# SnakeOnex/vit-is-all-you-need

Measured on AMD Instinct MI355X. Metric: images/sec ViT-B/16 224px bf16 fwd+bwd, higher is better.
Workload: dtype bf16; 1 GPU; ViT-B/16 224x224 bf16 forward+loss+backward, batch 256 per GPU (BASELINE configs[1]; configs[2] at 8 GPUs), random-init weights, 197 tokens, 79.44 M params; global_batch=256, parallelism=dp1

## Files before the change

vit-is-all-you-need_amd/csrc/attention.hip:

```cpp
#include "common.h"
#include "vitamd_internal.h"
#include <type_traits>

namespace {

constexpr int DH = 64;
constexpr int MAX_N = 512;
constexpr int MAX_N_LONG = 16384;
constexpr float NEG_BIG = -1.0e30f;

typedef LDS_AS bf16x4* lds_bf16x4_ptr;

__device__ __forceinline__ int swz(int row) { return (((row >> 1) & 1) << 2) | ((row >> 3) & 3); }

__device__ __forceinline__ void stage_tile(const __bf16* __restrict__ g, int ld, int N, int npad, char* lds, int wave, int lane, int nwaves = 4) {
  const int pieces = npad / 8;
  for (int pc = wave; pc < pieces; pc += nwaves) {
    const int row = pc * 8 + (lane >> 3);
    const int logical = (lane & 7) ^ swz(row);
    const int grow = min(row, N - 1);
    glds16(g + (size_t)grow * ld + logical * 8, lds + pc * 1024);
  }
}

__device__ __forceinline__ bf16x8 row_frag(const char* tile, int T, int kk, int lane) {
  const int rr = lane & 31;
  const int chunk = (2 * kk + (lane >> 5)) ^ swz(rr);
  return *(const bf16x8*)(tile + T * 4096 + rr * 128 + (chunk << 4));
}

__device__ __forceinline__ bf16x8 tr_frag(const char* tile, int T, int s, int dt, int lane) {
  const int h = lane >> 5, colhalf = (lane >> 4) & 1, qq = (lane >> 2) & 3, pp = lane & 3;
  const int chunk = 4 * dt + 2 * colhalf + (pp >> 1);
  bf16x4 part[2];
#pragma unroll
  for (int u = 0; u < 2; ++u) {
    const int rloc = 16 * s + 8 * u + 4 * h + qq;
    const int f = (((qq >> 1) & 1) << 2) | (2 * s + u);
    part[u] = __builtin_amdgcn_ds_read_tr16_b64_v4bf16((lds_bf16x4_ptr)(tile + T * 4096 + rloc * 128 + ((chunk ^ f) << 4) + (pp & 1) * 8));
  }
  return __builtin_shufflevector(part[0], part[1], 0, 1, 2, 3, 4, 5, 6, 7);
}

__device__ __forceinline__ bf16x8 acc_to_frag(const f32x16& x, int s) {
  bf16x8 f;
#pragma unroll
  for (int j = 0; j < 8; ++j) f[j] = (__bf16)x[8 * s + j];
  return f;
}

__device__ __forceinline__ void zero(f32x16& x) {
#pragma unroll
  for (int r = 0; r < 16; ++r) x[r] = 0.f;
}
__device__ __forceinline__ void zero(f32x16 (&x)[2]) {
#pragma unroll
  for (int dt = 0; dt < 2; ++dt) zero(x[dt]);
}

__device__ __forceinline__ void load_lane_frags(const __bf16* __restrict__ g, int ld, int N, int r0, int lane, bf16x8 (&f)[4]) {
  const int row = min(r0 + (lane & 31), N - 1);
  const __bf16* p = g + (size_t)row * ld + 8 * (lane >> 5);
#pragma unroll
  for (int kk = 0; kk < 4; ++kk) f[kk] = *(const bf16x8*)(p + 16 * kk);
}

__device__ __forceinline__ int acc_row(int reg, int lane) { return (reg & 3) + 8 * (reg >> 2) + 4 * (lane >> 5); }
__device__ __forceinline__ float fast_exp2(float x) { return __builtin_amdgcn_exp2f(x); }
__device__ __forceinline__ float max16(const f32x16& v) {
  float a = fmaxf(fmaxf(v[0], v[1]), fmaxf(v[2], v[3])), b = fmaxf(fmaxf(v[4], v[5]), fmaxf(v[6], v[7]));
  float c = fmaxf(fmaxf(v[8], v[9]), fmaxf(v[10], v[11])), d = fmaxf(fmaxf(v[12], v[13]), fmaxf(v[14], v[15]));
  return fmaxf(fmaxf(a, b), fmaxf(c, d));
}

__device__ __forceinline__ void store_rows_T(__bf16* __restrict__ g, int ld, int N, int r0, int lane, const f32x16 (&acc)[2], float scale) {
  const int row = r0 + (lane & 31);
  if (row >= N) return;
  __bf16* p = g + (size_t)row * ld + 4 * (lane >> 5);
#pragma unroll
  for (int dt = 0; dt < 2; ++dt)
#pragma unroll
    for (int u = 0; u < 4; ++u) {
      u32x2 o = {pack_bf16x2(acc[dt][4 * u] * scale, acc[dt][4 * u + 1] * scale),
                 pack_bf16x2(acc[dt][4 * u + 2] * scale, acc[dt][4 * u + 3] * scale)};
      *(u32x2*)(p + 32 * dt + 8 * u) = o;
    }
}

template <int ROWS = 32, bool RES = false>
__device__ __forceinline__ void store_rows_T_img(__bf16* __restrict__ g, int ld, int N, int r0, int lane, const f32x16 (&acc)[2], float scale, char* img,
                                                 float* colacc = nullptr, const float* __restrict__ xi = nullptr, float* __restrict__ xo = nullptr,
                                                 int ldx = 0) {
  const int rr = lane & 31, h = lane >> 5;
  constexpr int ITS = ROWS / 8;
  int pass = 0;
#pragma unroll
  do {
    f32x4 r[ITS][2];
    if constexpr (RES) {
#pragma unroll
      for (int it = 0; it < ITS; ++it) {
        const int row = (lane >> 3) + 8 * it, pc = lane & 7;
        const float* px = xi + (size_t)min(r0 + ROWS * pass + row, N - 1) * ldx + 8 * (pc ^ (row & 7));
        r[it][0] = *(const f32x4*)px;
        r[it][1] = *(const f32x4*)(px + 4);
      }
    }
    if (ROWS == 32 || (rr >> 4) == pass) {
#pragma unroll
      for (int dt = 0; dt < 2; ++dt)
#pragma unroll
        for (int u = 0; u < 4; ++u) {
          u32x2 o = {pack_bf16x2(acc[dt][4 * u] * scale, acc[dt][4 * u + 1] * scale),
                     pack_bf16x2(acc[dt][4 * u + 2] * scale, acc[dt][4 * u + 3] * scale)};
          *(u32x2*)(img + (rr & (ROWS - 1)) * 128 + (((4 * dt + u) ^ (rr & 7)) << 4) + h * 8) = o;
        }
    }
#pragma unroll
    for (int it = 0; it < ITS; ++it) {
      const int row = (lane >> 3) + 8 * it, pc = lane & 7;
      const u32x4 v = *(const u32x4*)(img + row * 128 + pc * 16);
      const int grow = r0 + ROWS * pass + row;
      if (grow < N) {
        const int col = 8 * (pc ^ (row & 7));
        *(u32x4*)(g + (size_t)grow * ld + col) = v;
        if constexpr (RES) {
          f32x4 o0 = {r[it][0][0] + bf16lo(v[0]), r[it][0][1] + bf16hi(v[0]), r[it][0][2] + bf16lo(v[1]), r[it][0][3] + bf16hi(v[1])};
          f32x4 o1 = {r[it][1][0] + bf16lo(v[2]), r[it][1][1] + bf16hi(v[2]), r[it][1][2] + bf16lo(v[3]), r[it][1][3] + bf16hi(v[3])};
          float* po = xo + (size_t)grow * ldx + col;
          *(f32x4*)po = o0;
          *(f32x4*)(po + 4) = o1;
        }
      }
    }
  } while (ROWS == 16 && ++pass < 2);
  if constexpr (ROWS == 32) {
    if (colacc) {
      const int chunk = lane >> 3, within = (lane & 7) * 2;
      const int nrows = min(32, N - r0);
      float sacc = 0.f;
      for (int row = 0; row < nrows; ++row)
        sacc += bf2f(*(const __bf16*)(img + row * 128 + ((chunk ^ (row & 7)) << 4) + within));
      *colacc += sacc;
    }
  }
}

struct AttnArgs {
  const __bf16* qkv;
  __bf16* o;
  float* lse2;
  const __bf16* d_o;
  __bf16* dqkv;
  float* delta;
  float* dbias;
  int B, N, H;
  int causal;
  float scale_log2e;
  float scale;
  unsigned drop_thresh;
  float drop_scale;
  unsigned seed_lo, seed_hi;
  const float* resid_in;
  float* resid_out;
  int nq;
};

struct HeadAddr {
  int b, hh, N, D3, D;
  const __bf16* qbase;
};
template <typename Idx>
__device__ __forceinline__ HeadAddr head_addr(const __bf16* qkv, int N, int H, Idx head) {
  const int b = head / H, hh = head % H, D3 = 3 * H * DH, D = H * DH;
  return {b, hh, N, D3, D, qkv + (size_t)b * N * D3 + hh * DH};
}
__device__ __forceinline__ size_t stat_index(int b, int H, int hh, int N, int row) { return ((size_t)b * H + hh) * N + row; }

__device__ __forceinline__ float attn_keep(const AttnArgs& a, int bh, int query, int key) {
  const unsigned long long idx = ((unsigned long long)bh * a.N + query) * a.N + key;
  return dropout_keep(idx, a.seed_lo, a.seed_hi, a.drop_thresh, a.drop_scale);
}

template <bool DROP>
__global__ __launch_bounds__(256) void attn_fwd_kernel(const AttnArgs a) {
  extern __shared__ __attribute__((aligned(16))) char smem[];
  const int lane = threadIdx.x & 63, wave = __builtin_amdgcn_readfirstlane(threadIdx.x >> 6);
  const auto [b, hh, N, D3, D, qbase] = head_addr(a.qkv, a.N, a.H, blockIdx.x);
  const int nt = (N + 31) / 32, npad = nt * 32;
  char* ktile = smem;
  char* vtile = smem + npad * 128;
  stage_tile(qbase + D, D3, N, npad, ktile, wave, lane);
  stage_tile(qbase + 2 * D, D3, N, npad, vtile, wave, lane);
  asm volatile("s_waitcnt vmcnt(0)" ::: "memory");
  __syncthreads();

  const float c = a.scale_log2e;
  for (int qb = wave; qb < nt; qb += 4) {
    const int q0 = qb * 32;
    const int qrow = q0 + (lane & 31);
    bf16x8 qf[4];
    load_lane_frags(qbase, D3, N, q0, lane, qf);
    f32x16 oacc[2];
    zero(oacc);
    float m = NEG_BIG, l = 0.f;
    const int t_end = a.causal ? min(nt, qb + 1) : nt;
    for (int T = 0; T < t_end; ++T) {
      f32x16 s;
      zero(s);
#pragma unroll
      for (int kk = 0; kk < 4; ++kk) s = __builtin_amdgcn_mfma_f32_32x32x16_bf16(row_frag(ktile, T, kk, lane), qf[kk], s, 0, 0, 0);
      if (32 * T + 32 > N || (a.causal && T == qb)) {
#pragma unroll
        for (int r = 0; r < 16; ++r) {
          const int key = 32 * T + acc_row(r, lane);
          if (!(key < N && (!a.causal || key <= qrow))) s[r] = NEG_BIG;
        }
      }
      float tmax = max16(s);
      tmax = fmaxf(tmax, __shfl_xor(tmax, 32, 64)) * c;
      const float mnew = fmaxf(m, tmax);
      const float alpha = fast_exp2(m - mnew);
      m = mnew;
      float psum = 0.f;
#pragma unroll
      for (int r = 0; r < 16; ++r) {
        s[r] = fast_exp2(__builtin_fmaf(s[r], c, -mnew));
        psum += s[r];
        if constexpr (DROP) s[r] *= attn_keep(a, blockIdx.x, min(qrow, N - 1), min(32 * T + acc_row(r, lane), N - 1));
      }
      l = l * alpha + psum;
#pragma unroll
      for (int dt = 0; dt < 2; ++dt)
#pragma unroll
        for (int r = 0; r < 16; ++r) oacc[dt][r] *= alpha;
#pragma unroll
      for (int sidx = 0; sidx < 2; ++sidx) {
        const bf16x8 pf = acc_to_frag(s, sidx);
#pragma unroll
        for (int dt = 0; dt < 2; ++dt)
          oacc[dt] = __builtin_amdgcn_mfma_f32_32x32x16_bf16(tr_frag(vtile, T, sidx, dt, lane), pf, oacc[dt], 0, 0, 0);
      }
    }
    l += __shfl_xor(l, 32, 64);
    const float inv = 1.0f / l;
    store_rows_T(a.o + (size_t)b * N * D + hh * DH, D, N, q0, lane, oacc, inv);
    if (lane < 32 && qrow < N) a.lse2[stat_index(b, a.H, hh, N, qrow)] = m + log2f(l);
  }
}

template <int NKT, bool DROP, bool CAUSAL, bool RES = false>
__global__ __launch_bounds__(256, 2) void attn_fwd_small_kernel(const AttnArgs a) {
  extern __shared__ __attribute__((aligned(16))) char smem[];
  const int lane = threadIdx.x & 63, wave = __builtin_amdgcn_readfirstlane(threadIdx.x >> 6);
  const int head = blockIdx.x;
  const auto [b, hh, N, D3, D, qbase] = head_addr(a.qkv, a.N, a.H, head);
  constexpr int nt = NKT, npad = NKT * 32;
  char* ktile = smem;
  char* vtile = smem + npad * 128;
  char* oimg = smem + 2 * npad * 128 + wave * 4096;
  stage_tile(qbase + D, D3, N, npad, ktile, wave, lane);
  stage_tile(qbase + 2 * D, D3, N, npad, vtile, wave, lane);
  const int wrot = (wave + head) & 3;
  bf16x8 qf[4], qf2[4];
  load_lane_frags(qbase, D3, N, wrot * 32, lane, qf);
  if (wrot + 4 < nt) load_lane_frags(qbase, D3, N, wrot * 32 + 128, lane, qf2);
  else {
#pragma unroll
    for (int kk = 0; kk < 4; ++kk) qf2[kk] = qf[kk];
  }
  asm volatile("s_waitcnt vmcnt(0)" ::: "memory");
#pragma unroll
  for (int kk = 0; kk < 4; ++kk) asm volatile("" : "+v"(qf[kk]), "+v"(qf2[kk]));
  __syncthreads();

  const float c = a.scale_log2e;
  for (int qb = wrot; qb < nt; qb += 4) {
    const int q0 = qb * 32;
    const int qrow = q0 + (lane & 31);
    if (qb != wrot) {
#pragma unroll
      for (int kk = 0; kk < 4; ++kk) qf[kk] = qf2[kk];
    }
    const int t_end = CAUSAL ? qb + 1 : nt;
    f32x16 s[NKT];
    float mx = NEG_BIG;
#pragma unroll
    for (int T = 0; T < NKT; ++T) {
      if (T < t_end) {
#pragma unroll
        for (int r = 0; r < 16; ++r) s[T][r] = 0.f;
#pragma unroll
        for (int kk = 0; kk < 4; ++kk) s[T] = __builtin_amdgcn_mfma_f32_32x32x16_bf16(row_frag(ktile, T, kk, lane), qf[kk], s[T], 0, 0, 0);
        if (32 * T + 32 > N || (CAUSAL && T == qb)) {
#pragma unroll
          for (int r = 0; r < 16; ++r) {
            const int key = 32 * T + acc_row(r, lane);
            if (!(key < N && (!CAUSAL || key <= qrow))) s[T][r] = NEG_BIG;
          }
        }
        mx = fmaxf(mx, max16(s[T]));
      }
    }
    mx = fmaxf(mx, __shfl_xor(mx, 32, 64));
    const float mc = mx * c;
    float l = 0.f;
    f32x16 oacc[2];
#pragma unroll
    for (int dt = 0; dt < 2; ++dt)
#pragma unroll
      for (int r = 0; r < 16; ++r) oacc[dt][r] = 0.f;
#pragma unroll
    for (int T = 0; T < NKT; ++T) {
      if (T < t_end) {
#pragma unroll
        for (int r = 0; r < 16; ++r) {
          float pexp = fast_exp2(__builtin_fmaf(s[T][r], c, -mc));
          l += pexp;
          if constexpr (DROP) pexp *= attn_keep(a, head, min(qrow, N - 1), min(32 * T + acc_row(r, lane), N - 1));
          s[T][r] = pexp;
        }
#pragma unroll
        for (int sidx = 0; sidx < 2; ++sidx) {
          const bf16x8 pf = acc_to_frag(s[T], sidx);
#pragma unroll
          for (int dt = 0; dt < 2; ++dt)
            oacc[dt] = __builtin_amdgcn_mfma_f32_32x32x16_bf16(tr_frag(vtile, T, sidx, dt, lane), pf, oacc[dt], 0, 0, 0);
        }
      }
    }
    l += __shfl_xor(l, 32, 64);
    const float inv = 1.0f / l;
    if constexpr (RES)
      store_rows_T_img<32, true>(a.o + (size_t)b * N * D + hh * DH, D, N, q0, lane, oacc, inv, oimg, nullptr, a.resid_in + (size_t)b * N * D + hh * DH,
                                 a.resid_out + (size_t)b * N * D + hh * DH, D);
    else
      store_rows_T_img(a.o + (size_t)b * N * D + hh * DH, D, N, q0, lane, oacc, inv, oimg);
    if (lane < 32 && qrow < N) a.lse2[stat_index(b, a.H, hh, N, qrow)] = mc + log2f(l);
  }
}

template <int NKT, bool RES, bool KEEP = false>
__global__ __launch_bounds__(512, 4) void attn_fwd_small8_kernel(const AttnArgs a) {
  extern __shared__ __attribute__((aligned(16))) char smem[];
  const int lane = threadIdx.x & 63, wave = __builtin_amdgcn_readfirstlane(threadIdx.x >> 6);
  const int head = blockIdx.x;
  const auto [b, hh, N, D3, D, qbase] = head_addr(a.qkv, a.N, a.H, head);
  constexpr int nt = NKT, npad = NKT * 32;
  char* ktile = smem;
  char* vtile = smem + npad * 128;
  char* oimg = smem + 2 * npad * 128 + wave * 2048;
  stage_tile(qbase + D, D3, N, npad, ktile, wave, lane, 8);
  stage_tile(qbase + 2 * D, D3, N, npad, vtile, wave, lane, 8);
  const int qb = (wave + head) & 7;
  bool active = qb < nt;
  if constexpr (KEEP) active = qb * 32 < a.nq;
  bf16x8 qf[4];
  load_lane_frags(qbase, D3, N, (active ? qb : 0) * 32, lane, qf);
  asm volatile("s_waitcnt vmcnt(0)" ::: "memory");
#pragma unroll
  for (int kk = 0; kk < 4; ++kk) asm volatile("" : "+v"(qf[kk]));
  __syncthreads();
  if (!active) return;
  const float c = a.scale_log2e;
  const int q0 = qb * 32;
  const int qrow = q0 + (lane & 31);
  float m = NEG_BIG, l = 0.f;
  f32x16 oacc[2];
  zero(oacc);
#pragma unroll 1
  for (int T = 0; T < NKT; ++T) {
    f32x16 st;
    zero(st);
#pragma unroll
    for (int kk = 0; kk < 4; ++kk) st = __builtin_amdgcn_mfma_f32_32x32x16_bf16(row_frag(ktile, T, kk, lane), qf[kk], st, 0, 0, 0);
    if (32 * T + 32 > N) {
#pragma unroll
      for (int r = 0; r < 16; ++r)
        if (!(32 * T + acc_row(r, lane) < N)) st[r] = NEG_BIG;
    }
    float mt = max16(st);
    mt = fmaxf(mt, __shfl_xor(mt, 32, 64));
    const float mn = fmaxf(m, mt);
    const float alpha = fast_exp2((m - mn) * c);
    m = mn;
    const float mc = mn * c;
    float lt = 0.f;
#pragma unroll
    for (int r = 0; r < 16; ++r) {
      const float pexp = fast_exp2(__builtin_fmaf(st[r], c, -mc));
      lt += pexp;
      st[r] = pexp;
    }
    l = l * alpha + lt;
    if (T > 0) {
#pragma unroll
      for (int dt = 0; dt < 2; ++dt)
#pragma unroll
        for (int r = 0; r < 16; ++r) oacc[dt][r] *= alpha;
    }
#pragma unroll
    for (int sidx = 0; sidx < 2; ++sidx) {
      const bf16x8 pf = acc_to_frag(st, sidx);
#pragma unroll
      for (int dt = 0; dt < 2; ++dt)
        oacc[dt] = __builtin_amdgcn_mfma_f32_32x32x16_bf16(tr_frag(vtile, T, sidx, dt, lane), pf, oacc[dt], 0, 0, 0);
    }
  }
  l += __shfl_xor(l, 32, 64);
  const float mc = m * c;
  const float inv = 1.0f / l;
  if constexpr (KEEP) {
    store_rows_T_img<16>(a.o + (size_t)b * a.nq * D + hh * DH, D, a.nq, q0, lane, oacc, inv, oimg);
    if (lane < 32 && qrow < a.nq) a.lse2[stat_index(b, a.H, hh, N, qrow)] = mc + log2f(l);
    return;
  }
  if constexpr (RES)
    store_rows_T_img<16, true>(a.o + (size_t)b * N * D + hh * DH, D, N, q0, lane, oacc, inv, oimg, nullptr, a.resid_in + (size_t)b * N * D + hh * DH,
                               a.resid_out + (size_t)b * N * D + hh * DH, D);
  else
    store_rows_T_img<16>(a.o + (size_t)b * N * D + hh * DH, D, N, q0, lane, oacc, inv, oimg);
  if (lane < 32 && qrow < N) a.lse2[stat_index(b, a.H, hh, N, qrow)] = mc + log2f(l);
}

template <bool DROP, bool CAUSAL>
__global__ __launch_bounds__(256, 2) void attn_bwd_dq_kernel(const AttnArgs a) {
  extern __shared__ __attribute__((aligned(16))) char smem[];
  const int lane = threadIdx.x & 63, wave = __builtin_amdgcn_readfirstlane(threadIdx.x >> 6);
  const auto [b, hh, N, D3, D, qbase] = head_addr(a.qkv, a.N, a.H, blockIdx.x);
  const int nt = (N + 31) / 32, npad = nt * 32;
  char* ktile = smem;
  char* vtile = smem + npad * 128;
  char* oimg = smem + 2 * npad * 128 + wave * 4096;
  stage_tile(qbase + D, D3, N, npad, ktile, wave, lane);
  stage_tile(qbase + 2 * D, D3, N, npad, vtile, wave, lane);
  asm volatile("s_waitcnt vmcnt(0)" ::: "memory");
  __syncthreads();

  const float c = a.scale_log2e;
  const __bf16* obase = a.o + (size_t)b * N * D + hh * DH;
  const __bf16* dobase = a.d_o + (size_t)b * N * D + hh * DH;
  float csum_q = 0.f;
  for (int qb = (wave + blockIdx.x) & 3; qb < nt; qb += 4) {
    const int q0 = qb * 32;
    const int qrow = q0 + (lane & 31);
    bf16x8 qf[4], dof[4], of[4];
    load_lane_frags(qbase, D3, N, q0, lane, qf);
    load_lane_frags(dobase, D, N, q0, lane, dof);
    load_lane_frags(obase, D, N, q0, lane, of);
    float delta = 0.f;
#pragma unroll
    for (int kk = 0; kk < 4; ++kk)
#pragma unroll
      for (int j = 0; j < 8; ++j) delta += (float)dof[kk][j] * (float)of[kk][j];
    delta += __shfl_xor(delta, 32, 64);
    const size_t stat = stat_index(b, a.H, hh, N, min(qrow, N - 1));
    const float lse2 = a.lse2[stat];
    if (lane < 32 && qrow < N) a.delta[stat] = delta;

    f32x16 dq[2];
    zero(dq);
    const int t_end = CAUSAL ? min(nt, qb + 1) : nt;
    for (int T = 0; T < t_end; ++T) {
      f32x16 s, dp;
      zero(s);
      zero(dp);
#pragma unroll
      for (int kk = 0; kk < 4; ++kk) {
        s = __builtin_amdgcn_mfma_f32_32x32x16_bf16(row_frag(ktile, T, kk, lane), qf[kk], s, 0, 0, 0);
        dp = __builtin_amdgcn_mfma_f32_32x32x16_bf16(row_frag(vtile, T, kk, lane), dof[kk], dp, 0, 0, 0);
      }
#pragma unroll
      for (int r = 0; r < 16; ++r) {
        const float pexp = fast_exp2(__builtin_fmaf(s[r], c, -lse2));
        float dpr = dp[r];
        if constexpr (DROP) dpr *= attn_keep(a, blockIdx.x, min(qrow, N - 1), min(32 * T + acc_row(r, lane), N - 1));
        s[r] = pexp * (dpr - delta);
      }
      if (32 * T + 32 > N || (CAUSAL && T == qb)) {
#pragma unroll
        for (int r = 0; r < 16; ++r) {
          const int key = 32 * T + acc_row(r, lane);
          if (!(key < N && (!CAUSAL || key <= qrow))) s[r] = 0.f;
        }
      }
#pragma unroll
      for (int sidx = 0; sidx < 2; ++sidx) {
        const bf16x8 dsf = acc_to_frag(s, sidx);
#pragma unroll
        for (int dt = 0; dt < 2; ++dt)
          dq[dt] = __builtin_amdgcn_mfma_f32_32x32x16_bf16(tr_frag(ktile, T, sidx, dt, lane), dsf, dq[dt], 0, 0, 0);
      }
    }
    store_rows_T_img(a.dqkv + (size_t)b * N * D3 + hh * DH, D3, N, q0, lane, dq, a.scale, oimg, a.dbias ? &csum_q : nullptr);
  }
  if (a.dbias) atomicAdd(a.dbias + hh * DH + lane, csum_q);
}

template <int NT, int NQT = NT, bool LIM = false>
__global__ __launch_bounds__(256, 2) void attn_bwd_dq_pipe_kernel(const AttnArgs a) {
  extern __shared__ __attribute__((aligned(16))) char smem[];
  const int lane = threadIdx.x & 63, wave = __builtin_amdgcn_readfirstlane(threadIdx.x >> 6);
  const int head = blockIdx.x;
  const auto [b, hh, N, D3, D, qbase] = head_addr(a.qkv, a.N, a.H, head);
  constexpr int nt = NT, npad = NT * 32;
  char* ktile = smem;
  char* vtile = smem + npad * 128;
  char* oimg = smem + 2 * npad * 128 + wave * 4096;
  stage_tile(qbase + D, D3, N, npad, ktile, wave, lane);
  stage_tile(qbase + 2 * D, D3, N, npad, vtile, wave, lane);
  int nq = N;
  if constexpr (LIM) nq = a.nq;
  const __bf16* obase = a.o + (size_t)b * nq * D + hh * DH;
  const __bf16* dobase = a.d_o + (size_t)b * nq * D + hh * DH;
  asm volatile("s_waitcnt vmcnt(0)" ::: "memory");
  __syncthreads();

  const float c = a.scale_log2e;
  float csum_q = 0.f;
  for (int qb = (wave + head) & 3; qb < nt; qb += 4) {
    const int q0 = qb * 32;
    const int qrow = q0 + (lane & 31);
    if constexpr (LIM) {
      if (qb >= NQT) {
        __bf16* zp = a.dqkv + (size_t)b * N * D3 + hh * DH + 8 * (lane & 7);
#pragma unroll
        for (int it = 0; it < 4; ++it) {
          const int row = q0 + (lane >> 3) + 8 * it;
          if (row < N) *(u32x4*)(zp + (size_t)row * D3) = (u32x4){0u, 0u, 0u, 0u};
        }
        continue;
      }
    }
    bf16x8 qf[4], dof[4];
    float delta = 0.f;
    {
      bf16x8 of[4];
      load_lane_frags(qbase, D3, N, q0, lane, qf);
      load_lane_frags(dobase, D, nq, q0, lane, dof);
      load_lane_frags(obase, D, nq, q0, lane, of);
      if constexpr (LIM) {
        if (qrow >= nq) {
#pragma unroll
          for (int kk = 0; kk < 4; ++kk)
#pragma unroll
            for (int j = 0; j < 8; ++j) dof[kk][j] = (__bf16)0.f;
        }
      }
#pragma unroll
      for (int kk = 0; kk < 4; ++kk)
#pragma unroll
        for (int j = 0; j < 8; ++j) delta += (float)dof[kk][j] * (float)of[kk][j];
    }
    delta += __shfl_xor(delta, 32, 64);
    const size_t stat = stat_index(b, a.H, hh, N, min(qrow, nq - 1));
    float lse2 = a.lse2[stat];
    if constexpr (LIM) lse2 = qrow < nq ? lse2 : 1.0e30f;
    if (lane < 32 && qrow < nq) a.delta[stat] = delta;

    f32x16 dq[2];
#pragma unroll
    for (int dt = 0; dt < 2; ++dt)
#pragma unroll
      for (int r = 0; r < 16; ++r) dq[dt][r] = 0.f;
    bf16x8 kr[2][4], vr[2][4];
    f32x16 sb[2], dpb[2];
    auto products = [&](int buf) {
#pragma unroll
      for (int r = 0; r < 16; ++r) { sb[buf][r] = 0.f; dpb[buf][r] = 0.f; }
#pragma unroll
      for (int kk = 0; kk < 4; ++kk) {
        sb[buf] = __builtin_amdgcn_mfma_f32_32x32x16_bf16(kr[buf][kk], qf[kk], sb[buf], 0, 0, 0);
        dpb[buf] = __builtin_amdgcn_mfma_f32_32x32x16_bf16(vr[buf][kk], dof[kk], dpb[buf], 0, 0, 0);
      }
    };
#pragma unroll
    for (int kk = 0; kk < 4; ++kk) { kr[0][kk] = row_frag(ktile, 0, kk, lane); vr[0][kk] = row_frag(vtile, 0, kk, lane); }
    if (NT > 1) {
#pragma unroll
      for (int kk = 0; kk < 4; ++kk) { kr[1][kk] = row_frag(ktile, 1, kk, lane); vr[1][kk] = row_frag(vtile, 1, kk, lane); }
    }
    products(0);
#pragma unroll
    for (int T = 0; T < NT; ++T) {
      const int cur = T & 1, nxt = cur ^ 1;
      bf16x8 ktr[2][2];
#pragma unroll
      for (int sidx = 0; sidx < 2; ++sidx)
#pragma unroll
        for (int dt = 0; dt < 2; ++dt) ktr[sidx][dt] = tr_frag(ktile, T, sidx, dt, lane);
      __builtin_amdgcn_sched_barrier(0);
      if (T + 1 < NT) products(nxt);
      if (T + 2 < NT) {
#pragma unroll
        for (int kk = 0; kk < 4; ++kk) { kr[cur][kk] = row_frag(ktile, T + 2, kk, lane); vr[cur][kk] = row_frag(vtile, T + 2, kk, lane); }
      }
#pragma unroll
      for (int r = 0; r < 16; ++r) {
        const float pexp = fast_exp2(__builtin_fmaf(sb[cur][r], c, -lse2));
        sb[cur][r] = pexp * (dpb[cur][r] - delta);
      }
      if (T == NT - 1 && 32 * T + 32 > N) {
#pragma unroll
        for (int r = 0; r < 16; ++r)
          if (!(32 * T + acc_row(r, lane) < N)) sb[cur][r] = 0.f;
      }
#pragma unroll
      for (int sidx = 0; sidx < 2; ++sidx) {
        const bf16x8 dsf = acc_to_frag(sb[cur], sidx);
#pragma unroll
        for (int dt = 0; dt < 2; ++dt) dq[dt] = __builtin_amdgcn_mfma_f32_32x32x16_bf16(ktr[sidx][dt], dsf, dq[dt], 0, 0, 0);
      }
    }
    store_rows_T_img(a.dqkv + (size_t)b * N * D3 + hh * DH, D3, N, q0, lane, dq, a.scale, oimg, a.dbias ? &csum_q : nullptr);
  }
  if (a.dbias) atomicAdd(a.dbias + hh * DH + lane, csum_q);
}

template <bool DROP, bool CAUSAL>
__global__ __launch_bounds__(256, 2) void attn_bwd_dkv_kernel(const AttnArgs a) {
  extern __shared__ __attribute__((aligned(16))) char smem[];
  const int lane = threadIdx.x & 63, wave = __builtin_amdgcn_readfirstlane(threadIdx.x >> 6);
  const auto [b, hh, N, D3, D, qbase] = head_addr(a.qkv, a.N, a.H, blockIdx.x);
  const int nt = (N + 31) / 32, npad = nt * 32;
  char* qtile = smem;
  char* dotile = smem + npad * 128;
  float* lse_s = (float*)(smem + 2 * npad * 128);
  float* delta_s = lse_s + npad;
  char* oimg = smem + 2 * npad * 128 + 2 * npad * 4 + wave * 4096;
  const __bf16* dobase = a.d_o + (size_t)b * N * D + hh * DH;
  stage_tile(qbase, D3, N, npad, qtile, wave, lane);
  stage_tile(dobase, D, N, npad, dotile, wave, lane);
  for (int i = threadIdx.x; i < npad; i += 256) {
    const size_t stat = stat_index(b, a.H, hh, N, min(i, N - 1));
    lse_s[i] = a.lse2[stat];
    delta_s[i] = a.delta[stat];
  }
  asm volatile("s_waitcnt vmcnt(0)" ::: "memory");
  __syncthreads();

  const float c = a.scale_log2e;
  float csum_k = 0.f, csum_v = 0.f;
  for (int kb = (wave + blockIdx.x) & 3; kb < nt; kb += 4) {
    const int k0 = kb * 32;
    const int krow = k0 + (lane & 31);
    bf16x8 kf[4], vf[4];
    load_lane_frags(qbase + D, D3, N, k0, lane, kf);
    load_lane_frags(qbase + 2 * D, D3, N, k0, lane, vf);
    f32x16 dk[2], dv[2];
    zero(dk);
    zero(dv);
    const int t_beg = CAUSAL ? kb : 0;
    for (int T = t_beg; T < nt; ++T) {
      f32x16 s, dp;
      zero(s);
      zero(dp);
#pragma unroll
      for (int kk = 0; kk < 4; ++kk) {
        s = __builtin_amdgcn_mfma_f32_32x32x16_bf16(row_frag(qtile, T, kk, lane), kf[kk], s, 0, 0, 0);
        dp = __builtin_amdgcn_mfma_f32_32x32x16_bf16(row_frag(dotile, T, kk, lane), vf[kk], dp, 0, 0, 0);
      }
      f32x16 pmat;
#pragma unroll
      for (int u = 0; u < 4; ++u) {
        const int qr = 32 * T + 8 * u + 4 * (lane >> 5);
        const f32x4 lse4 = *(const f32x4*)(lse_s + qr);
        const f32x4 del4 = *(const f32x4*)(delta_s + qr);
#pragma unroll
        for (int i = 0; i < 4; ++i) {
          const int r = 4 * u + i;
          const float pexp = fast_exp2(__builtin_fmaf(s[r], c, -lse4[i]));
          float keep = 1.0f;
          if constexpr (DROP) keep = attn_keep(a, blockIdx.x, min(qr + i, N - 1), min(krow, N - 1));
          pmat[r] = pexp * keep;
          s[r] = pexp * (dp[r] * keep - del4[i]);
        }
        if (32 * T + 32 > N || k0 + 32 > N || (CAUSAL && T == kb)) {
#pragma unroll
          for (int i = 0; i < 4; ++i) {
            const int r = 4 * u + i, query = qr + i;
            if (!(query < N && krow < N && (!CAUSAL || krow <= query))) { pmat[r] = 0.f; s[r] = 0.f; }
          }
        }
      }
#pragma unroll
      for (int sidx = 0; sidx < 2; ++sidx) {
        const bf16x8 pf = acc_to_frag(pmat, sidx);
        const bf16x8 dsf = acc_to_frag(s, sidx);
#pragma unroll
        for (int dt = 0; dt < 2; ++dt) {
          dv[dt] = __builtin_amdgcn_mfma_f32_32x32x16_bf16(tr_frag(dotile, T, sidx, dt, lane), pf, dv[dt], 0, 0, 0);
          dk[dt] = __builtin_amdgcn_mfma_f32_32x32x16_bf16(tr_frag(qtile, T, sidx, dt, lane), dsf, dk[dt], 0, 0, 0);
        }
      }
    }
    __bf16* dbase = a.dqkv + (size_t)b * N * D3 + hh * DH;
    store_rows_T_img(dbase + D, D3, N, k0, lane, dk, a.scale, oimg, a.dbias ? &csum_k : nullptr);
    store_rows_T_img(dbase + 2 * D, D3, N, k0, lane, dv, 1.0f, oimg, a.dbias ? &csum_v : nullptr);
  }
  if (a.dbias) {
    atomicAdd(a.dbias + D + hh * DH + lane, csum_k);
    atomicAdd(a.dbias + 2 * D + hh * DH + lane, csum_v);
  }
}

template <int NT, int NQT = NT, bool LIM = false>
__global__ __launch_bounds__(256, 2) void attn_bwd_dkv_pipe_kernel(const AttnArgs a) {
  extern __shared__ __attribute__((aligned(16))) char smem[];
  const int lane = threadIdx.x & 63, wave = __builtin_amdgcn_readfirstlane(threadIdx.x >> 6);
  const int head = blockIdx.x;
  const int b = head / a.H, hh = head % a.H;
  const int N = a.N, D3 = 3 * a.H * DH, D = a.H * DH;
  constexpr int nt = NT, npad = NQT * 32;
  int nq = N;
  if constexpr (LIM) nq = a.nq;
  char* qtile = smem;
  char* dotile = smem + npad * 128;
  float* lse_s = (float*)(smem + 2 * npad * 128);
  float* delta_s = lse_s + npad;
  char* oimg = smem + 2 * npad * 128 + 2 * npad * 4 + wave * 4096;
  const __bf16* qbase = a.qkv + (size_t)b * N * D3 + hh * DH;
  const __bf16* dobase = a.d_o + (size_t)b * nq * D + hh * DH;
  stage_tile(qbase, D3, N, npad, qtile, wave, lane);
  stage_tile(dobase, D, nq, npad, dotile, wave, lane);
  for (int i = threadIdx.x; i < npad; i += 256) {
    const size_t stat = ((size_t)b * a.H + hh) * N + min(i, nq - 1);
    lse_s[i] = i < nq ? a.lse2[stat] : 1.0e30f;
    delta_s[i] = a.delta[stat];
  }
  asm volatile("s_waitcnt vmcnt(0)" ::: "memory");
  __syncthreads();

  const float c = a.scale_log2e;
  float csum_k = 0.f, csum_v = 0.f;
  for (int kb = (wave + head) & 3; kb < nt; kb += 4) {
    const int k0 = kb * 32;
    bf16x8 kf[4], vf[4];
    load_lane_frags(qbase + D, D3, N, k0, lane, kf);
    load_lane_frags(qbase + 2 * D, D3, N, k0, lane, vf);
    f32x16 dk[2], dv[2];
    zero(dk);
    zero(dv);
    bf16x8 qr[4], dor[4];
    f32x16 sb, dpb;
    auto products = [&]() {
      zero(sb);
      zero(dpb);
#pragma unroll
      for (int kk = 0; kk < 4; ++kk) {
        sb = __builtin_amdgcn_mfma_f32_32x32x16_bf16(qr[kk], kf[kk], sb, 0, 0, 0);
        dpb = __builtin_amdgcn_mfma_f32_32x32x16_bf16(dor[kk], vf[kk], dpb, 0, 0, 0);
      }
    };
#pragma unroll
    for (int kk = 0; kk < 4; ++kk) { qr[kk] = row_frag(qtile, 0, kk, lane); dor[kk] = row_frag(dotile, 0, kk, lane); }
    products();
    if (NQT > 1) {
#pragma unroll
      for (int kk = 0; kk < 4; ++kk) { qr[kk] = row_frag(qtile, 1, kk, lane); dor[kk] = row_frag(dotile, 1, kk, lane); }
    }
#pragma unroll
    for (int T = 0; T < NQT; ++T) {
      bf16x8 dotr[2][2], qtr[2][2];
      f32x4 lse4[4], del4[4];
#pragma unroll
      for (int sidx = 0; sidx < 2; ++sidx)
#pragma unroll
        for (int dt = 0; dt < 2; ++dt) { dotr[sidx][dt] = tr_frag(dotile, T, sidx, dt, lane); qtr[sidx][dt] = tr_frag(qtile, T, sidx, dt, lane); }
      __builtin_amdgcn_sched_barrier(0);
#pragma unroll
      for (int u = 0; u < 4; ++u) {
        const int qr0 = 32 * T + 8 * u + 4 * (lane >> 5);
        lse4[u] = *(const f32x4*)(lse_s + qr0);
        del4[u] = *(const f32x4*)(delta_s + qr0);
      }
      f32x16 pmat;
#pragma unroll
      for (int u = 0; u < 4; ++u)
#pragma unroll
        for (int i = 0; i < 4; ++i) {
          const int r = 4 * u + i;
          const float pexp = fast_exp2(__builtin_fmaf(sb[r], c, -lse4[u][i]));
          pmat[r] = pexp;
          sb[r] = pexp * (dpb[r] - del4[u][i]);
        }
#pragma unroll
      for (int sidx = 0; sidx < 2; ++sidx) {
        const bf16x8 pf = acc_to_frag(pmat, sidx);
        const bf16x8 dsf = acc_to_frag(sb, sidx);
#pragma unroll
        for (int dt = 0; dt < 2; ++dt) {
          dv[dt] = __builtin_amdgcn_mfma_f32_32x32x16_bf16(dotr[sidx][dt], pf, dv[dt], 0, 0, 0);
          dk[dt] = __builtin_amdgcn_mfma_f32_32x32x16_bf16(qtr[sidx][dt], dsf, dk[dt], 0, 0, 0);
        }
      }
      if (T + 1 < NQT) products();
      if (T + 2 < NQT) {
#pragma unroll
        for (int kk = 0; kk < 4; ++kk) { qr[kk] = row_frag(qtile, T + 2, kk, lane); dor[kk] = row_frag(dotile, T + 2, kk, lane); }
      }
    }
    __bf16* dbase = a.dqkv + (size_t)b * N * D3 + hh * DH;
    store_rows_T_img(dbase + D, D3, N, k0, lane, dk, a.scale, oimg, a.dbias ? &csum_k : nullptr);
    store_rows_T_img(dbase + 2 * D, D3, N, k0, lane, dv, 1.0f, oimg, a.dbias ? &csum_v : nullptr);
  }
  if (a.dbias) {
    atomicAdd(a.dbias + D + hh * DH + lane, csum_k);
    atomicAdd(a.dbias + 2 * D + hh * DH + lane, csum_v);
  }
}

constexpr int CH = 512;

template <bool DROP>
__global__ __launch_bounds__(256) void attn_fwd_long_kernel(const AttnArgs a) {
  extern __shared__ __attribute__((aligned(16))) char smem[];
  const int lane = threadIdx.x & 63, wave = __builtin_amdgcn_readfirstlane(threadIdx.x >> 6);
  const auto [b, hh, N, D3, D, qbase] = head_addr(a.qkv, a.N, a.H, blockIdx.x);
  const int nt = (N + 31) / 32;
  char* ktile = smem;
  char* vtile = smem + CH * 128;
  const int qb = blockIdx.y * 4 + wave;
  const bool active = qb < nt;
  const int q0 = qb * 32, qrow = q0 + (lane & 31);
  const float c = a.scale_log2e;
  bf16x8 qf[4];
  if (active) load_lane_frags(qbase, D3, N, q0, lane, qf);
  f32x16 oacc[2];
  zero(oacc);
  float m = NEG_BIG, l = 0.f;
  const int t_end = a.causal ? min(nt, qb + 1) : nt;
  for (int k0 = 0; k0 < N; k0 += CH) {
    const int rows = min(CH, N - k0), ntc = (rows + 31) / 32;
    __syncthreads();
    stage_tile(qbase + D + (size_t)k0 * D3, D3, rows, ntc * 32, ktile, wave, lane);
    stage_tile(qbase + 2 * D + (size_t)k0 * D3, D3, rows, ntc * 32, vtile, wave, lane);
    asm volatile("s_waitcnt vmcnt(0)" ::: "memory");
    __syncthreads();
    if (!active) continue;
    for (int T = 0; T < ntc && k0 / 32 + T < t_end; ++T) {
      const int key0 = k0 + 32 * T;
      f32x16 s;
      zero(s);
#pragma unroll
      for (int kk = 0; kk < 4; ++kk) s = __builtin_amdgcn_mfma_f32_32x32x16_bf16(row_frag(ktile, T, kk, lane), qf[kk], s, 0, 0, 0);
      if (key0 + 32 > N || (a.causal && key0 / 32 == qb)) {
#pragma unroll
        for (int r = 0; r < 16; ++r) {
          const int key = key0 + acc_row(r, lane);
          if (!(key < N && (!a.causal || key <= qrow))) s[r] = NEG_BIG;
        }
      }
      float tmax = max16(s);
      tmax = fmaxf(tmax, __shfl_xor(tmax, 32, 64)) * c;
      const float mnew = fmaxf(m, tmax);
      const float alpha = fast_exp2(m - mnew);
      m = mnew;
      float psum = 0.f;
#pragma unroll
      for (int r = 0; r < 16; ++r) {
        s[r] = fast_exp2(__builtin_fmaf(s[r], c, -mnew));
        psum += s[r];
        if constexpr (DROP) s[r] *= attn_keep(a, blockIdx.x, min(qrow, N - 1), min(key0 + acc_row(r, lane), N - 1));
      }
      l = l * alpha + psum;
#pragma unroll
      for (int dt = 0; dt < 2; ++dt)
#pragma unroll
        for (int r = 0; r < 16; ++r) oacc[dt][r] *= alpha;
#pragma unroll
      for (int sidx = 0; sidx < 2; ++sidx) {
        const bf16x8 pf = acc_to_frag(s, sidx);
#pragma unroll
        for (int dt = 0; dt < 2; ++dt)
          oacc[dt] = __builtin_amdgcn_mfma_f32_32x32x16_bf16(tr_frag(vtile, T, sidx, dt, lane), pf, oacc[dt], 0, 0, 0);
      }
    }
  }
  if (!active) return;
  l += __shfl_xor(l, 32, 64);
  const float inv = 1.0f / l;
  store_rows_T(a.o + (size_t)b * N * D + hh * DH, D, N, q0, lane, oacc, inv);
  if (lane < 32 && qrow < N) a.lse2[stat_index(b, a.H, hh, N, qrow)] = m + log2f(l);
}

template <bool DROP>
__global__ __launch_bounds__(256) void attn_bwd_dq_long_kernel(const AttnArgs a) {
  extern __shared__ __attribute__((aligned(16))) char smem[];
  const int lane = threadIdx.x & 63, wave = __builtin_amdgcn_readfirstlane(threadIdx.x >> 6);
  const auto [b, hh, N, D3, D, qbase] = head_addr(a.qkv, a.N, a.H, blockIdx.x);
  const int nt = (N + 31) / 32;
  char* ktile = smem;
  char* vtile = smem + CH * 128;
  char* oimg = smem + 2 * CH * 128 + wave * 4096;
  const __bf16* obase = a.o + (size_t)b * N * D + hh * DH;
  const __bf16* dobase = a.d_o + (size_t)b * N * D + hh * DH;
  const int qb = blockIdx.y * 4 + wave;
  const bool active = qb < nt;
  const int q0 = qb * 32, qrow = q0 + (lane & 31);
  const float c = a.scale_log2e;
  bf16x8 qf[4], dof[4];
  float delta = 0.f, lse2 = 0.f;
  if (active) {
    bf16x8 of[4];
    load_lane_frags(qbase, D3, N, q0, lane, qf);
    load_lane_frags(dobase, D, N, q0, lane, dof);
    load_lane_frags(obase, D, N, q0, lane, of);
#pragma unroll
    for (int kk = 0; kk < 4; ++kk)
#pragma unroll
      for (int j = 0; j < 8; ++j) delta += (float)dof[kk][j] * (float)of[kk][j];
    delta += __shfl_xor(delta, 32, 64);
    const size_t stat = stat_index(b, a.H, hh, N, min(qrow, N - 1));
    lse2 = a.lse2[stat];
    if (lane < 32 && qrow < N) a.delta[stat] = delta;
  }
  f32x16 dq[2];
  zero(dq);
  const int t_end = a.causal ? min(nt, qb + 1) : nt;
  for (int k0 = 0; k0 < N; k0 += CH) {
    const int rows = min(CH, N - k0), ntc = (rows + 31) / 32;
    __syncthreads();
    stage_tile(qbase + D + (size_t)k0 * D3, D3, rows, ntc * 32, ktile, wave, lane);
    stage_tile(qbase + 2 * D + (size_t)k0 * D3, D3, rows, ntc * 32, vtile, wave, lane);
    asm volatile("s_waitcnt vmcnt(0)" ::: "memory");
    __syncthreads();
    if (!active) continue;
    for (int T = 0; T < ntc && k0 / 32 + T < t_end; ++T) {
      const int key0 = k0 + 32 * T;
      f32x16 s, dp;
      zero(s);
      zero(dp);
#pragma unroll
      for (int kk = 0; kk < 4; ++kk) {
        s = __builtin_amdgcn_mfma_f32_32x32x16_bf16(row_frag(ktile, T, kk, lane), qf[kk], s, 0, 0, 0);
        dp = __builtin_amdgcn_mfma_f32_32x32x16_bf16(row_frag(vtile, T, kk, lane), dof[kk], dp, 0, 0, 0);
      }
#pragma unroll
      for (int r = 0; r < 16; ++r) {
        const float pexp = fast_exp2(__builtin_fmaf(s[r], c, -lse2));
        float dpr = dp[r];
        if constexpr (DROP) dpr *= attn_keep(a, blockIdx.x, min(qrow, N - 1), min(key0 + acc_row(r, lane), N - 1));
        s[r] = pexp * (dpr - delta);
      }
      if (key0 + 32 > N || (a.causal && key0 / 32 == qb)) {
#pragma unroll
        for (int r = 0; r < 16; ++r) {
          const int key = key0 + acc_row(r, lane);
          if (!(key < N && (!a.causal || key <= qrow))) s[r] = 0.f;
        }
      }
#pragma unroll
      for (int sidx = 0; sidx < 2; ++sidx) {
        const bf16x8 dsf = acc_to_frag(s, sidx);
#pragma unroll
        for (int dt = 0; dt < 2; ++dt)
          dq[dt] = __builtin_amdgcn_mfma_f32_32x32x16_bf16(tr_frag(ktile, T, sidx, dt, lane), dsf, dq[dt], 0, 0, 0);
      }
    }
  }
  float csum_q = 0.f;
  if (active) store_rows_T_img(a.dqkv + (size_t)b * N * D3 + hh * DH, D3, N, q0, lane, dq, a.scale, oimg, a.dbias ? &csum_q : nullptr);
  if (a.dbias && active) atomicAdd(a.dbias + hh * DH + lane, csum_q);
}

template <bool DROP>
__global__ __launch_bounds__(256) void attn_bwd_dkv_long_kernel(const AttnArgs a) {
  extern __shared__ __attribute__((aligned(16))) char smem[];
  const int lane = threadIdx.x & 63, wave = __builtin_amdgcn_readfirstlane(threadIdx.x >> 6);
  const auto [b, hh, N, D3, D, qbase] = head_addr(a.qkv, a.N, a.H, blockIdx.x);
  const int nt = (N + 31) / 32;
  char* qtile = smem;
  char* dotile = smem + CH * 128;
  float* lse_s = (float*)(smem + 2 * CH * 128);
  float* delta_s = lse_s + CH;
  char* oimg = smem + 2 * CH * 128 + 2 * CH * 4 + wave * 4096;
  const __bf16* dobase = a.d_o + (size_t)b * N * D + hh * DH;
  const int kb = blockIdx.y * 4 + wave;
  const bool active = kb < nt;
  const int k0 = kb * 32, krow = k0 + (lane & 31);
  const float c = a.scale_log2e;
  bf16x8 kf[4], vf[4];
  if (active) {
    load_lane_frags(qbase + D, D3, N, k0, lane, kf);
    load_lane_frags(qbase + 2 * D, D3, N, k0, lane, vf);
  }
  f32x16 dk[2], dv[2];
#pragma unroll
  for (int dt = 0; dt < 2; ++dt)
#pragma unroll
    for (int r = 0; r < 16; ++r) { dk[dt][r] = 0.f; dv[dt][r] = 0.f; }
  const int t_beg = a.causal ? kb : 0;
  for (int r0 = 0; r0 < N; r0 += CH) {
    const int rows = min(CH, N - r0), ntc = (rows + 31) / 32;
    __syncthreads();
    stage_tile(qbase + (size_t)r0 * D3, D3, rows, ntc * 32, qtile, wave, lane);
    stage_tile(dobase + (size_t)r0 * D, D, rows, ntc * 32, dotile, wave, lane);
    for (int i = threadIdx.x; i < ntc * 32; i += 256) {
      const size_t stat = stat_index(b, a.H, hh, N, min(r0 + i, N - 1));
      lse_s[i] = a.lse2[stat];
      delta_s[i] = a.delta[stat];
    }
    asm volatile("s_waitcnt vmcnt(0)" ::: "memory");
    __syncthreads();
    if (!active) continue;
    for (int T = 0; T < ntc; ++T) {
      const int Tg = r0 / 32 + T;
      if (Tg < t_beg) continue;
      f32x16 s, dp;
#pragma unroll
      for (int r = 0; r < 16; ++r) { s[r] = 0.f; dp[r] = 0.f; }
#pragma unroll
      for (int kk = 0; kk < 4; ++kk) {
        s = __builtin_amdgcn_mfma_f32_32x32x16_bf16(row_frag(qtile, T, kk, lane), kf[kk], s, 0, 0, 0);
        dp = __builtin_amdgcn_mfma_f32_32x32x16_bf16(row_frag(dotile, T, kk, lane), vf[kk], dp, 0, 0, 0);
      }
      f32x16 pmat;
#pragma unroll
      for (int u = 0; u < 4; ++u) {
        const int ql = 32 * T + 8 * u + 4 * (lane >> 5);
        const f32x4 lse4 = *(const f32x4*)(lse_s + ql);
        const f32x4 del4 = *(const f32x4*)(delta_s + ql);
#pragma unroll
        for (int i = 0; i < 4; ++i) {
          const int r = 4 * u + i;
          const float pexp = fast_exp2(__builtin_fmaf(s[r], c, -lse4[i]));
          float keep = 1.0f;
          if constexpr (DROP) keep = attn_keep(a, blockIdx.x, min(r0 + ql + i, N - 1), min(krow, N - 1));
          pmat[r] = pexp * keep;
          s[r] = pexp * (dp[r] * keep - del4[i]);
        }
        if (r0 + 32 * T + 32 > N || k0 + 32 > N || (a.causal && Tg == kb)) {
#pragma unroll
          for (int i = 0; i < 4; ++i) {
            const int r = 4 * u + i, query = r0 + ql + i;
            if (!(query < N && krow < N && (!a.causal || krow <= query))) { pmat[r] = 0.f; s[r] = 0.f; }
          }
        }
      }
#pragma unroll
      for (int sidx = 0; sidx < 2; ++sidx) {
        const bf16x8 pf = acc_to_frag(pmat, sidx);
        const bf16x8 dsf = acc_to_frag(s, sidx);
#pragma unroll
        for (int dt = 0; dt < 2; ++dt) {
          dv[dt] = __builtin_amdgcn_mfma_f32_32x32x16_bf16(tr_frag(dotile, T, sidx, dt, lane), pf, dv[dt], 0, 0, 0);
          dk[dt] = __builtin_amdgcn_mfma_f32_32x32x16_bf16(tr_frag(qtile, T, sidx, dt, lane), dsf, dk[dt], 0, 0, 0);
        }
      }
    }
  }
  if (!active) return;
  float csum_k = 0.f, csum_v = 0.f;
  __bf16* dbase = a.dqkv + (size_t)b * N * D3 + hh * DH;
  store_rows_T_img(dbase + D, D3, N, k0, lane, dk, a.scale, oimg, a.dbias ? &csum_k : nullptr);
  store_rows_T_img(dbase + 2 * D, D3, N, k0, lane, dv, 1.0f, oimg, a.dbias ? &csum_v : nullptr);
  if (a.dbias) {
    atomicAdd(a.dbias + D + hh * DH + lane, csum_k);
    atomicAdd(a.dbias + 2 * D + hh * DH + lane, csum_v);
  }
}

int make_args(AttnArgs& out, bool bwd, const void* qkv, const void* o, const float* lse2, const void* d_o, void* dqkv, float* delta, float* dbias, int B,
              int N, int H, int head_dim, int causal, float p, unsigned long long seed, int nq = 0) {
  if (head_dim != DH || B <= 0 || N <= 0 || H <= 0 || N > MAX_N_LONG) return VITAMD_ERR_SHAPE;
  if (!qkv || !o || !lse2 || (bwd && (!d_o || !dqkv || !delta))) return VITAMD_ERR_ARG;
  const DropoutParams d = dropout_params(p, seed);
  if (!d.ok) return VITAMD_ERR_ARG;
  AttnArgs a{};
  a.qkv = (const __bf16*)qkv;
  a.o = (__bf16*)o;
  a.lse2 = (float*)lse2;
  a.d_o = (const __bf16*)d_o;
  a.dqkv = (__bf16*)dqkv;
  a.delta = delta;
  a.dbias = dbias;
  a.B = B;
  a.N = N;
  a.H = H;
  a.causal = causal;
  a.scale = 0.125f;
  a.scale_log2e = 0.125f * 1.4426950408889634f;
  a.drop_thresh = d.thresh;
  a.drop_scale = d.scale;
  a.seed_lo = d.seed_lo;
  a.seed_hi = d.seed_hi;
  a.nq = nq;
  out = a;
  return VITAMD_OK;
}

int launched(int e) { return e ? e : hipGetLastError() == hipSuccess ? VITAMD_OK : VITAMD_ERR_LAUNCH; }

template <int LO, int HI, typename F>
int with_tiles(int v, F f) {
  if constexpr (LO > HI) return VITAMD_ERR_SHAPE;
  else return v == LO ? f(std::integral_constant<int, LO>{}) : with_tiles<LO + 1, HI>(v, f);
}
template <typename F>
int with_flag(bool v, F f) { return v ? f(std::true_type{}) : f(std::false_type{}); }
#define CONST_OF(arg) decltype(arg)::value

template <int NT, int NQT, bool LIM>
int launch_bwd_pipe(const AttnArgs& a, hipStream_t stream) {
  if constexpr (NQT > NT) return VITAMD_ERR_SHAPE;
  else {
    const dim3 grid(a.B * a.H), block(256);
// ... 111 lines not shown
```

Before: 9363 images/sec.

## Pipeline attention K/V and Q/dO tile staging with per-tile vmcnt waits

Replaces the monolithic stage-everything-then-sync prologue in the small forward attention kernel and the backward dK/dV kernel with buffer-resource loads issued per 32-row tile. Each compute step waits only on the vmcnt count for the tile it needs, followed by a barrier. The backward kernel also prefetches the next K/V row fragments while the current results are stored, and loads lse/delta into registers in the same batch as the tile loads. This aims to overlap global-to-LDS latency with MFMA work. In exchange it adds more barriers and depends on exact counting of outstanding memory operations, which is fragile.

```diff
diff --git a/vit-is-all-you-need_amd/csrc/attention.hip b/vit-is-all-you-need_amd/csrc/attention.hip
--- a/vit-is-all-you-need_amd/csrc/attention.hip
+++ b/vit-is-all-you-need_amd/csrc/attention.hip
@@ -64,6 +64,41 @@
 #pragma unroll
   for (int kk = 0; kk < 4; ++kk) f[kk] = *(const bf16x8*)(p + 16 * kk);
 }
+
+#define ATTN_WAIT_VM(n) asm volatile("s_waitcnt vmcnt(%0)" ::"n"(n) : "memory")
+__device__ __forceinline__ void wait_vm_left(int left) {
+  switch (left) {
+    case 0: ATTN_WAIT_VM(0); break;
+    case 1: ATTN_WAIT_VM(1); break;
+    case 2: ATTN_WAIT_VM(2); break;
+    case 3: ATTN_WAIT_VM(3); break;
+    case 4: ATTN_WAIT_VM(4); break;
+    case 5: ATTN_WAIT_VM(5); break;
+    case 6: ATTN_WAIT_VM(6); break;
+    case 7: ATTN_WAIT_VM(7); break;
+    case 8: ATTN_WAIT_VM(8); break;
+    case 9: ATTN_WAIT_VM(9); break;
+    default: ATTN_WAIT_VM(10); break;
+  }
+}
+__device__ __forceinline__ void stage_piece(srd_t srd, unsigned soff, int ldb, int N, unsigned lds, int pc, int lane) {
+  const int row = pc * 8 + (lane >> 3);
+  const int logical = (lane & 7) ^ swz(row);
+  asm_glds16(srd, lds + pc * 1024, (unsigned)(min(row, N - 1) * ldb + logical * 16), soff);
+}
+__device__ __forceinline__ void lane_frags_asm(srd_t srd, unsigned soff, int ldb, int N, int r0, int lane, bf16x8 (&f)[4]) {
+  const unsigned voff = (unsigned)(min(r0 + (lane & 31), N - 1) * ldb + 16 * (lane >> 5));
+  asm volatile("s_nop 4\n\tbuffer_load_dwordx4 %0, %4, %5, %6 offen\n\tbuffer_load_dwordx4 %1, %4, %5, %6 offen offset:32\n\t"
+               "buffer_load_dwordx4 %2, %4, %5, %6 offen offset:64\n\tbuffer_load_dwordx4 %3, %4, %5, %6 offen offset:96"
+               : "=&v"(f[0]), "=&v"(f[1]), "=&v"(f[2]), "=&v"(f[3]) : "v"(voff), "s"(srd), "s"(soff) : "memory");
+}
+__device__ __forceinline__ float stat_asm(srd_t srd, int index) {
+  float r;
+  asm volatile("s_nop 4\n\tbuffer_load_dword %0, %1, %2, 0 offen" : "=v"(r) : "v"((unsigned)(index * 4)), "s"(srd) : "memory");
+  return r;
+}
+#define ATTN_WAIT_VM_FRAGS(n, f) asm volatile("s_waitcnt vmcnt(%4)" : "+v"(f[0]), "+v"(f[1]), "+v"(f[2]), "+v"(f[3]) : "n"(n) : "memory")
+__host__ __device__ constexpr int bwd_left(int nt, int t) { return t + 1 >= nt ? 0 : 2 * (nt - 1 - t); }
 
 __device__ __forceinline__ int acc_row(int reg, int lane) { return (reg & 3) + 8 * (reg >> 2) + 4 * (lane >> 5); }
 __device__ __forceinline__ float fast_exp2(float x) { return __builtin_amdgcn_exp2f(x); }
@@ -350,18 +385,28 @@
   char* ktile = smem;
   char* vtile = smem + npad * 128;
   char* oimg = smem + 2 * npad * 128 + wave * 2048;
-  stage_tile(qbase + D, D3, N, npad, ktile, wave, lane, 8);
-  stage_tile(qbase + 2 * D, D3, N, npad, vtile, wave, lane, 8);
   const int qb = (wave + head) & 7;
   bool active = qb < nt;
   if constexpr (KEEP) active = qb * 32 < a.nq;
+  const srd_t sqkv = make_srd(qbase, (size_t)(N - 1) * D3 * 2 + 4 * D + 128);
+  auto request_pieces = [&]() {
+    const unsigned soff = wave < 4 ? 2 * D : 4 * D, lds = lds_addr(wave < 4 ? ktile : vtile);
+#pragma unroll
+    for (int T = 0; T < NKT; ++T) stage_piece(sqkv, soff, D3 * 2, N, lds, 4 * T + (wave & 3), lane);
+  };
+  if (!active) {
+    request_pieces();
+#pragma unroll 1
+    for (int T = 0; T < NKT; ++T) {
+      wait_vm_left(NKT - 1 - T);
+      __builtin_amdgcn_s_barrier();
+    }
+    return;
+  }
   bf16x8 qf[4];
-  load_lane_frags(qbase, D3, N, (active ? qb : 0) * 32, lane, qf);
-  asm volatile("s_waitcnt vmcnt(0)" ::: "memory");
-#pragma unroll
-  for (int kk = 0; kk < 4; ++kk) asm volatile("" : "+v"(qf[kk]));
-  __syncthreads();
-  if (!active) return;
+  lane_frags_asm(sqkv, 0u, D3 * 2, N, qb * 32, lane, qf);
+  request_pieces();
+  ATTN_WAIT_VM_FRAGS(NKT - 1, qf);
   const float c = a.scale_log2e;
   const int q0 = qb * 32;
   const int qrow = q0 + (lane & 31);
@@ -370,6 +415,8 @@
   zero(oacc);
 #pragma unroll 1
   for (int T = 0; T < NKT; ++T) {
+    wait_vm_left(NKT - 1 - T);
+    __builtin_amdgcn_s_barrier();
     f32x16 st;
     zero(st);
 #pragma unroll
@@ -721,23 +768,65 @@
   char* oimg = smem + 2 * npad * 128 + 2 * npad * 4 + wave * 4096;
   const __bf16* qbase = a.qkv + (size_t)b * N * D3 + hh * DH;
   const __bf16* dobase = a.d_o + (size_t)b * nq * D + hh * DH;
-  stage_tile(qbase, D3, N, npad, qtile, wave, lane);
-  stage_tile(dobase, D, nq, npad, dotile, wave, lane);
-  for (int i = threadIdx.x; i < npad; i += 256) {
-    const size_t stat = ((size_t)b * a.H + hh) * N + min(i, nq - 1);
-    lse_s[i] = i < nq ? a.lse2[stat] : 1.0e30f;
-    delta_s[i] = a.delta[stat];
-  }
-  asm volatile("s_waitcnt vmcnt(0)" ::: "memory");
-  __syncthreads();
+  const int kb0 = (wave + head) & 3;
+  const srd_t sqkv = make_srd(qbase, (size_t)(N - 1) * D3 * 2 + 4 * D + 128);
+  const srd_t sdo = make_srd(dobase, (size_t)(nq - 1) * D * 2 + 128);
+  const srd_t slse = make_srd(a.lse2 + ((size_t)b * a.H + hh) * N, (size_t)N * 4), sdel = make_srd(a.delta + ((size_t)b * a.H + hh) * N, (size_t)N * 4);
+  auto request_pieces = [&]() {
+#pragma unroll
+    for (int T = 0; T < NQT; ++T) {
+      stage_piece(sqkv, 0u, D3 * 2, N, lds_addr(qtile), 4 * T + wave, lane);
+      stage_piece(sdo, 0u, D * 2, nq, lds_addr(dotile), 4 * T + wave, lane);
+    }
+  };
+  bf16x8 kf[4], vf[4];
+  auto request_rows = [&](int kb) {
+    lane_frags_asm(sqkv, 2 * D, D3 * 2, N, kb * 32, lane, kf);
+    lane_frags_asm(sqkv, 4 * D, D3 * 2, N, kb * 32, lane, vf);
+  };
+  bool first = !LIM && kb0 < nt;
+  if constexpr (LIM) {
+    stage_tile(qbase, D3, N, npad, qtile, wave, lane);
+    stage_tile(dobase, D, nq, npad, dotile, wave, lane);
+    for (int i = threadIdx.x; i < npad; i += 256) {
+      const size_t stat = ((size_t)b * a.H + hh) * N + min(i, nq - 1);
+      lse_s[i] = i < nq ? a.lse2[stat] : 1.0e30f;
+      delta_s[i] = a.delta[stat];
+    }
+    asm volatile("s_waitcnt vmcnt(0)" ::: "memory");
+    __syncthreads();
+  } else {
+    static_assert(LIM || NQT * 32 <= 256, "one lse / delta entry per thread");
+    const int si = threadIdx.x;
+    float lse_v = stat_asm(slse, min(si, nq - 1)), delta_v = stat_asm(sdel, min(si, nq - 1));
+    request_rows(min(kb0, nt - 1));
+    request_pieces();
+    asm volatile("s_waitcnt vmcnt(%10)"
+                 : "+v"(kf[0]), "+v"(kf[1]), "+v"(kf[2]), "+v"(kf[3]), "+v"(vf[0]), "+v"(vf[1]), "+v"(vf[2]), "+v"(vf[3]), "+v"(lse_v), "+v"(delta_v)
+                 : "n"(bwd_left(NQT, 1))
+                 : "memory");
+    if (si < npad) {
+      lse_s[si] = si < nq ? lse_v : 1.0e30f;
+      delta_s[si] = delta_v;
+    }
+    __syncthreads();
+    if (!first) {
+#pragma unroll
+      for (int T = 0; T + 2 < NQT; ++T) {
+        wait_vm_left(bwd_left(NQT, T + 2));
+        __builtin_amdgcn_s_barrier();
+      }
+    }
+  }
 
   const float c = a.scale_log2e;
   float csum_k = 0.f, csum_v = 0.f;
-  for (int kb = (wave + head) & 3; kb < nt; kb += 4) {
+  for (int kb = kb0; kb < nt; kb += 4) {
     const int k0 = kb * 32;
-    bf16x8 kf[4], vf[4];
-    load_lane_frags(qbase + D, D3, N, k0, lane, kf);
-    load_lane_frags(qbase + 2 * D, D3, N, k0, lane, vf);
+    if constexpr (LIM) {
+      load_lane_frags(qbase + D, D3, N, k0, lane, kf);
+      load_lane_frags(qbase + 2 * D, D3, N, k0, lane, vf);
+    }
     f32x16 dk[2], dv[2];
     zero(dk);
     zero(dv);
@@ -795,14 +884,26 @@
         }
       }
       if (T + 1 < NQT) products();
+      if (T + 2 < NQT && first) {
+        wait_vm_left(bwd_left(NQT, T + 2));
+        __builtin_amdgcn_s_barrier();
+      }
       if (T + 2 < NQT) {
 #pragma unroll
         for (int kk = 0; kk < 4; ++kk) { qr[kk] = row_frag(qtile, T + 2, kk, lane); dor[kk] = row_frag(dotile, T + 2, kk, lane); }
       }
     }
+    first = false;
+    const bool more = !LIM && kb + 4 < nt;
+    if (more) request_rows(kb + 4);
     __bf16* dbase = a.dqkv + (size_t)b * N * D3 + hh * DH;
     store_rows_T_img(dbase + D, D3, N, k0, lane, dk, a.scale, oimg, a.dbias ? &csum_k : nullptr);
     store_rows_T_img(dbase + 2 * D, D3, N, k0, lane, dv, 1.0f, oimg, a.dbias ? &csum_v : nullptr);
+    if (more)
+      asm volatile("s_waitcnt vmcnt(0)"
+                   : "+v"(kf[0]), "+v"(kf[1]), "+v"(kf[2]), "+v"(kf[3]), "+v"(vf[0]), "+v"(vf[1]), "+v"(vf[2]), "+v"(vf[3])
+                   :
+                   : "memory");
   }
   if (a.dbias) {
     atomicAdd(a.dbias + D + hh * DH + lane, csum_k);
```

Measured after the change: 9428 images/sec, median of 6. About the same (+0.7%).
